# yynil/RWKV_LM_EXT

Measured on AMD Instinct MI355X. Metric: WKV6 fwd+bwd tokens/sec/GPU (B=8,T=4096,C=2048) + %HBM roofline, higher is better.
Workload: dtype bf16

## Files before the change

### rwkv_lm_ext_amd/csrc/wkv6_chunk.hip

```cpp
#include <type_traits>
#include "wkv6_chunk.h"

namespace wkv6 {
namespace {

using namespace chunk;

constexpr int GRP_BYTES = NBLK * BLK_BYTES;
constexpr int CKX_BYTES = 4 * 4096;
constexpr int CONSUMER_STAGGER = 3;
constexpr int YRS = 144;
constexpr int YS_BYTES = GRP * YRS;

struct FwdRaw {
    uint2 pr[4], pk[4], pv[4], pw[4];
    float4 pe[4];
};
template <bool W_RAW, bool STATE_ONLY, bool AFF>
__device__ __forceinline__ void fwd_request_group(const ScanArgs& a, const int b, const int h, const int ntok, const int rev, const int grp, const int wv,
                                                  const int lane, FwdRaw& raw)
{
    const int c4 = lane & 15, tq = lane >> 4;
    const long base = (long)b * a.T * a.C + (long)h * HEAD;
    const TokAddr<AFF> tok(ntok, rev != 0);
    const int C_ = a.C;
    const unsigned span = ntok > 0 ? (unsigned)(ntok - 1) * a.C : 0u;
    const unsigned nb2 = ntok > 0 ? span * 2 + 128 : 0;
    const rsrc_t rs_r = make_rsrc(reinterpret_cast<const bf16_t*>(a.r) + base, nb2), rs_k = make_rsrc(reinterpret_cast<const bf16_t*>(a.k) + base, nb2);
    const rsrc_t rs_v = make_rsrc(reinterpret_cast<const bf16_t*>(a.v) + base, nb2);
    const rsrc_t rs_w = W_RAW ? make_rsrc(reinterpret_cast<const bf16_t*>(a.w) + base, nb2)
                              : make_rsrc(reinterpret_cast<const float*>(a.w) + base, ntok > 0 ? span * 4 + 256 : 0);
#pragma unroll
    for (int tt = 0; tt < 4; ++tt) {
        const int pl = wv * BLK + 4 * tq + tt, lp = tok.lane(pl, 4 * c4, C_);
        if constexpr (!STATE_ONLY) raw.pr[tt] = buf_load8(rs_r, tok.off(grp * GRP, pl, 4 * c4, C_, REV_R, lp) * 2);
        else raw.pr[tt] = make_uint2(0u, 0u);
        raw.pk[tt] = buf_load8(rs_k, tok.off(grp * GRP, pl, 4 * c4, C_, REV_K, lp) * 2);
        raw.pv[tt] = buf_load8(rs_v, tok.off(grp * GRP, pl, 4 * c4, C_, REV_V, lp) * 2);
        if constexpr (W_RAW) raw.pw[tt] = buf_load8(rs_w, tok.off(grp * GRP, pl, 4 * c4, C_, REV_W, lp) * 2);
        else raw.pe[tt] = buf_load16f(rs_w, tok.off(grp * GRP, pl, 4 * c4, C_, REV_W, lp) * 4);
    }
}
struct FwdChain {
    int b, ntok;
    int pb;
    bool chained_in;
    bool nx_valid;
    unsigned nx_bh;
    int nx_b, nx_ntok;
    bool nx_rev, nx_use_u;
};
__device__ __forceinline__ bool fwd_hw_wave_produces(int hw) { return hw >= 4; }
template <bool W_RAW, bool STATE_ONLY, bool ACC, bool GN, bool AFF, bool CLK = false, bool CHAIN = false, bool VARLEN = false>
__device__ __forceinline__ void chunk_fwd_body(const ScanArgs& a, const unsigned slot, const unsigned sslot, FwdRaw& raw, const FwdChain& ch = FwdChain{})
{
    [[maybe_unused]] const bool nxvalid = ch.nx_valid, chained_in = ch.chained_in, nx_use_u = ch.nx_use_u;
    [[maybe_unused]] const unsigned nxbh = ch.nx_bh;
    [[maybe_unused]] const int nxrev = ch.nx_rev, b_known = ch.b, ntok_known = ch.ntok, nxb = ch.nx_b, nxntok = ch.nx_ntok, pb = CHAIN ? ch.pb : 0;
    extern __shared__ __attribute__((aligned(16))) char smem[];
    const int tid = threadIdx.x, lane = tid & 63;
    const SplitConst spc = split_const();
    const int hwid = __builtin_amdgcn_readfirstlane(tid >> 6);
    const int part = a.split ? (int)(slot & 1) : 0;
    const int bh = a.split ? (int)(slot >> 1) : (CLK ? (int)(slot + 0u * (unsigned)(a.B * a.H)) : (int)slot);
    int wid, cidx;
    wid = a.split ? (hwid < 2 ? 2 * part + hwid : hwid + 2) : hwid;
    cidx = hwid;
    const bool producer = wid >= 4;
    const int wv = wid & 3;
    const int b = CHAIN ? b_known : (a.order ? a.order[bh / a.H] : bh / a.H), h = bh % a.H;
    const long base = VARLEN ? (long)a.tok_off[b] * a.C + (long)h * HEAD : (long)b * a.T * a.C + (long)h * HEAD;
    const bf16_t* const gr_ = reinterpret_cast<const bf16_t*>(a.r) + base;
    const bf16_t* const gk_ = reinterpret_cast<const bf16_t*>(a.k) + base;
    const bf16_t* const gv_ = reinterpret_cast<const bf16_t*>(a.v) + base;
    bf16_t* const gy_ = reinterpret_cast<bf16_t*>(a.y) + base;
    int ntok = a.T;
    if constexpr (CHAIN) ntok = ntok_known;
    else if (a.lens) ntok = min(max(a.lens[b], 0), a.T);
    const int ngrp = (ntok + GRP - 1) / GRP;
    const TokAddr<AFF> tok(a, b, ntok);
    const int C_ = a.C;
#ifdef WKV6_STAMP
    unsigned long long stamp_acc[6] = {0, 0, 0, 0, 0, 0}, ts0 = 0, ts1 = 0, ts2 = 0, ts3 = 0, ts4 = 0;
#endif
#ifdef WKV6_DEBUGBUF
    unsigned long long clk0 = 0, rtc0 = 0, clk1 = 0, rtc1 = 0;
    WKV6_CLK(clk0, rtc0);
#endif
    if constexpr (CLK) { if (hwid == 0) clock_stamp(a, slot, 0); }

    if (producer) {
        const int c4 = lane & 15, tq = lane >> 4;
        float uu[4] = {0.f, 0.f, 0.f, 0.f};
        if (a.use_u) io4<bf16_t>::load(reinterpret_cast<const bf16_t*>(a.u) + h * HEAD + 4 * c4, uu);
        uint2 (&pr)[4] = raw.pr, (&pk)[4] = raw.pk, (&pv)[4] = raw.pv, (&pw)[4] = raw.pw;
        float4 (&pe)[4] = raw.pe;
        float dtot[4] = {0.f, 0.f, 0.f, 0.f};
        const unsigned span = ntok > 0 ? (unsigned)(ntok - 1) * a.C : 0u;
        const rsrc_t rs_r = make_rsrc(gr_, ntok > 0 ? span * 2 + 128 : 0), rs_k = make_rsrc(gk_, ntok > 0 ? span * 2 + 128 : 0);
        const rsrc_t rs_v = make_rsrc(gv_, ntok > 0 ? span * 2 + 128 : 0);
        const rsrc_t rs_w = W_RAW ? make_rsrc(reinterpret_cast<const bf16_t*>(a.w) + base, ntok > 0 ? span * 2 + 128 : 0)
                                  : make_rsrc(reinterpret_cast<const float*>(a.w) + base, ntok > 0 ? span * 4 + 256 : 0);
        const int lp_in[4] = {tok.lane(wv * BLK + 4 * tq, 4 * c4, C_), tok.lane(wv * BLK + 4 * tq + 1, 4 * c4, C_),
                              tok.lane(wv * BLK + 4 * tq + 2, 4 * c4, C_), tok.lane(wv * BLK + 4 * tq + 3, 4 * c4, C_)};
        auto load_quad = [&](int grp, int tt) {
            {
                const int pl = wv * BLK + 4 * tq + tt;
                const unsigned ir = tok.off(grp * GRP, pl, 4 * c4, C_, REV_R, lp_in[tt]), ik = tok.off(grp * GRP, pl, 4 * c4, C_, REV_K, lp_in[tt]);
                const unsigned iv = tok.off(grp * GRP, pl, 4 * c4, C_, REV_V, lp_in[tt]), iw = tok.off(grp * GRP, pl, 4 * c4, C_, REV_W, lp_in[tt]);
                if constexpr (!STATE_ONLY) pr[tt] = buf_load8(rs_r, ir * 2);
                else pr[tt] = make_uint2(0u, 0u);
                pk[tt] = buf_load8(rs_k, ik * 2);
                pv[tt] = buf_load8(rs_v, iv * 2);
                if constexpr (W_RAW) pw[tt] = buf_load8(rs_w, iw * 2);
                else pe[tt] = buf_load16f(rs_w, iw * 4);
            }
        };
        auto load_group = [&](int grp) {
#pragma unroll
            for (int tt = 0; tt < 4; ++tt) load_quad(grp, tt);
        };
        auto prep_group = [&](int grp, int buf, const int ntok, const float (&uu)[4], auto&& request_next) {
            char* const bb = smem + buf * GRP_BYTES + wv * BLK_BYTES;
            float r[4][4], k[4][4], cs[4][4];
#pragma unroll
            for (int tt = 0; tt < 4; ++tt) {
                const bool valid = grp * GRP + wv * BLK + 4 * tq + tt < ntok;
                r[tt][0] = bf_lo(pr[tt].x); r[tt][1] = bf_hi(pr[tt].x); r[tt][2] = bf_lo(pr[tt].y); r[tt][3] = bf_hi(pr[tt].y);
                k[tt][0] = bf_lo(pk[tt].x); k[tt][1] = bf_hi(pk[tt].x); k[tt][2] = bf_lo(pk[tt].y); k[tt][3] = bf_hi(pk[tt].y);
                float lw[4];
                if constexpr (W_RAW) {
                    lw[0] = -LOG2E * exp2_fast(LOG2E * bf_lo(pw[tt].x)); lw[1] = -LOG2E * exp2_fast(LOG2E * bf_hi(pw[tt].x));
                    lw[2] = -LOG2E * exp2_fast(LOG2E * bf_lo(pw[tt].y)); lw[3] = -LOG2E * exp2_fast(LOG2E * bf_hi(pw[tt].y));
                } else {
                    lw[0] = pe[tt].x; lw[1] = pe[tt].y; lw[2] = pe[tt].z; lw[3] = pe[tt].w;
                    if (a.wkind == 2) {
#pragma unroll
                        for (int c = 0; c < 4; ++c) lw[c] = __builtin_amdgcn_logf(lw[c]);
                    } else {
#pragma unroll
                        for (int c = 0; c < 4; ++c) lw[c] *= LOG2E;
                    }
                }
#pragma unroll
                for (int c = 0; c < 4; ++c) {
                    const float l = valid ? fmaxf(lw[c], LW_MIN2) : 0.f;
                    cs[tt][c] = tt ? cs[tt - 1][c] + l : l;
                }
                if constexpr (!STATE_ONLY) {
                    float part = 0.f;
#pragma unroll
                    for (int c = 0; c < 4; ++c) part = fmaf(r[tt][c] * uu[c], k[tt][c], part);
                    part = row_sum16(part);
                    if (c4 == 0) *reinterpret_cast<float*>(bb + OFF_COEF + (4 * tq + tt) * 4) = part;
                }
                *reinterpret_cast<uint2*>(bb + A_V * ARR + (4 * tq + tt) * RSB + 8 * c4) = pv[tt];
            }
            __builtin_amdgcn_sched_barrier(0);
            request_next();
            float pre[4], c8[4], c16[4];
#pragma unroll
            for (int c = 0; c < 4; ++c) {
                float a_, b_;
                rows16(cs[3][c], a_, b_);
                float pfx = (tq & 1) ? a_ : 0.f;
                halves32(a_ + b_, a_, b_);
                pfx += (tq & 2) ? a_ : 0.f;
                pre[c] = pfx;
                c8[c] = a_;
                c16[c] = a_ + b_;
                dtot[c] += c16[c];
            }
            if (tq == 0) {
                *reinterpret_cast<float4*>(bb + OFF_E8 + 16 * c4) =
                    make_float4(exp2_fast(c8[0]), exp2_fast(c8[1]), exp2_fast(c8[2]), exp2_fast(c8[3]));
                *reinterpret_cast<float4*>(bb + OFF_E16M8 + 16 * c4) =
                    make_float4(exp2_fast(c16[0] - c8[0]), exp2_fast(c16[1] - c8[1]), exp2_fast(c16[2] - c8[2]), exp2_fast(c16[3] - c8[3]));
            }
#pragma unroll
            for (int tt = 0; tt < 4; ++tt) {
                float rh[4], kh[4];
#pragma unroll
                for (int c = 0; c < 4; ++c) {
                    const float cex = tt ? pre[c] + cs[tt - 1][c] : pre[c];
                    const float cin = pre[c] + cs[tt][c];
                    rh[c] = r[tt][c] * exp2_fast(cex - c8[c]);
                    kh[c] = k[tt][c] * exp2_fast(c8[c] - cin);
                }
                char* const row = bb + (4 * tq + tt) * RSB + 8 * c4;
                uint2 hi, lo;
                if constexpr (!STATE_ONLY) {
                    split4(rh, hi, lo, spc);
                    *reinterpret_cast<uint2*>(row + A_RH * ARR) = hi; *reinterpret_cast<uint2*>(row + A_RL * ARR) = lo;
                }
                split4(kh, hi, lo, spc);
                *reinterpret_cast<uint2*>(row + A_KH * ARR) = hi; *reinterpret_cast<uint2*>(row + A_KL * ARR) = lo;
            }
            if constexpr (!STATE_ONLY) {
                const int x = lane & 15, g = lane >> 4;
                f4v sc = {0.f, 0.f, 0.f, 0.f};
#pragma unroll
                for (int s = 0; s < 2; ++s) {
                    const int off = x * RSB + (32 * s + 8 * g) * 2;
                    const b8v kh = ld_b8(bb + A_KH * ARR + off), kl = ld_b8(bb + A_KL * ARR + off);
                    const b8v rh = ld_b8(bb + A_RH * ARR + off), rl = ld_b8(bb + A_RL * ARR + off);
                    sc = mfma32(kh, rh, sc);
                    sc = mfma32(kh, rl, sc);
                    sc = mfma32(kl, rh, sc);
                }
                const float cf = *reinterpret_cast<const float*>(bb + OFF_COEF + x * 4);
                float scm[4];
#pragma unroll
                for (int q = 0; q < 4; ++q) {
                    const int bt = 4 * g + q;
                    scm[q] = bt < x ? sc[q] : (bt == x ? cf : 0.f);
                }
                uint2 sh, sl;
                split4(scm, sh, sl, spc);
                *reinterpret_cast<uint4*>(bb + OFF_SC + lane * 16) = make_uint4(sh.x, sh.y, sl.x, sl.y);
            }
        };

        float uu_nx[4] = {0.f, 0.f, 0.f, 0.f};
        if constexpr (CHAIN) { if (nxvalid && nx_use_u) io4<bf16_t>::load(reinterpret_cast<const bf16_t*>(a.u) + (nxbh % (unsigned)a.H) * HEAD + 4 * c4, uu_nx); }
        if (!(CHAIN && chained_in)) {
            if (ngrp > 0) {
                load_group(0);
                prep_group(0, pb & 1, ntok, uu, [&]() { load_group(1); });
            }
            __syncthreads();
        }
        for (int grp = 0; grp + 1 < ngrp; ++grp) {
            WKV6_T(ts0);
#ifdef WKV6_STAMP
            asm volatile("" :: "v"(pr[0].x), "v"(pk[0].x), "v"(pv[0].x), "v"(pw[0].x), "v"(pr[3].x), "v"(pk[3].x), "v"(pv[3].x),
                         "v"(pw[3].x));
#endif
            WKV6_T(ts1);
            prep_group(grp + 1, (grp + 1 + pb) & 1, ntok, uu, [&]() { load_group(grp + 2); });
            WKV6_T(ts2);
            WKV6_T(ts3);
            __syncthreads();
            WKV6_T(ts4);
            WKV6_ACC(0, ts1, ts0); WKV6_ACC(1, ts2, ts1); WKV6_ACC(2, ts3, ts2); WKV6_ACC(3, ts4, ts3);
        }
        if constexpr (CHAIN) {
            if (nxvalid) {
                const int nxh = (int)(nxbh % (unsigned)a.H);
                fwd_request_group<W_RAW, STATE_ONLY, AFF>(a, nxb, nxh, nxntok, nxrev, 0, wv, lane, raw);
                prep_group(0, (ngrp + pb) & 1, nxntok, uu_nx, [&]() { fwd_request_group<W_RAW, STATE_ONLY, AFF>(a, nxb, nxh, nxntok, nxrev, 1, wv, lane, raw); });
            }
        }
        if (ngrp > 0) __syncthreads();
        if (a.dsum && tq == 0 && part == 0)
            *reinterpret_cast<float4*>(a.dsum + ((long)(b * a.H + h) * 4 + wv) * HEAD + 4 * c4) = make_float4(dtot[0], dtot[1], dtot[2], dtot[3]);
    } else {
        const int x = lane & 15, g = lane >> 4;
        f4v St[4];
#pragma unroll
        for (int it = 0; it < 4; ++it) {
            float t4[4] = {0.f, 0.f, 0.f, 0.f};
            if (a.s0) {
                const long so_ = (long)b * a.s0_bstride + ((long)h * HEAD + 16 * wv + x) * HEAD + tile_ch(it) + 8 * g;
                if (a.state_f32) io4<float>::load(reinterpret_cast<const float*>(a.s0) + so_, t4);
                else io4<bf16_t>::load(reinterpret_cast<const bf16_t*>(a.s0) + so_, t4);
            }
            St[it] = f4v{t4[0], t4[1], t4[2], t4[3]};
            asm volatile("" : "+v"(St[it]));
        }
        int troff = (4 * g + (x >> 2)) * RSB + 8 * (x & 3);
        int trow = (4 * g + (x >> 2)) * RSB + 16 * (x & 3);
        const rsrc_t rs_y = make_rsrc(a.y ? gy_ : nullptr, (!STATE_ONLY && a.y && ntok > 0) ? (unsigned)(ntok - 1) * a.C * 2u + 128u : 0u);
        const unsigned nst = VARLEN ? (unsigned)ngrp : ((unsigned)a.T + CKPT_TOK - 1) / CKPT_TOK;
        const int segs = a.ckpt_segs > 1 ? a.ckpt_segs : 1;
        const long ck_slot0 = VARLEN ? (long)h * a.ck_stride + a.ck_off[b] : ((long)((b / segs) * a.H + h) * segs + b % segs) * nst;
        const rsrc_t rs_ck = make_rsrc(a.ckpt ? a.ckpt + ck_slot0 * (HEAD * HEAD) : nullptr, a.ckpt ? nst * 16384u : 0u);
        const unsigned ystr = a.side_compact ? (unsigned)HEAD : (unsigned)a.C;
        const unsigned ych = a.side_compact ? 16u * (unsigned)cidx : 16u * (unsigned)wv;
        const rsrc_t rs_yf = make_rsrc(a.y_f32 ? a.y_f32 + (a.side_compact ? (long)sslot * a.T * HEAD : base) : nullptr,
                                       (a.y_f32 && !STATE_ONLY && ntok > 0) ? (unsigned)(ntok - 1) * ystr * 4u + 256u : 0u);
        const int lp_y = tok.lane(x, 16 * wv + 4 * g, C_), lp_ys = tok.lane(x, (int)ych + 4 * g, (int)ystr);
        [[maybe_unused]] uint4 acc_cur[NBLK] = {}, acc_nxt[NBLK] = {};
        auto acc_request = [&](int grp_, uint4 (&dst)[NBLK]) {
#pragma unroll
            for (int blk = 0; blk < NBLK; ++blk) {
                const unsigned idx = tok.off(grp_ * GRP + blk * BLK, x, 16 * wv + 4 * g, C_, REV_Y, lp_y);
                if (a.y_f32) {
                    const float4 t = buf_load16f(rs_yf, tok.off(grp_ * GRP + blk * BLK, x, (int)ych + 4 * g, (int)ystr, REV_Y, lp_ys) * 4u);
                    dst[blk] = make_uint4(__float_as_uint(t.x), __float_as_uint(t.y), __float_as_uint(t.z), __float_as_uint(t.w));
                } else {
                    const uint2 t = buf_load8(rs_y, idx * 2u);
                    dst[blk] = make_uint4(t.x, t.y, 0u, 0u);
                }
            }
        };
        auto acc_add = [&](const uint4& r, float (&o)[4]) {
            if (a.y_f32) { o[0] += __uint_as_float(r.x); o[1] += __uint_as_float(r.y); o[2] += __uint_as_float(r.z); o[3] += __uint_as_float(r.w); }
            else { o[0] += bf_lo(r.x); o[1] += bf_hi(r.x); o[2] += bf_lo(r.y); o[3] += bf_hi(r.y); }
        };
        if constexpr (ACC) {
            acc_request(0, acc_cur);
#pragma unroll
            for (int blk = 0; blk < NBLK; ++blk) asm volatile("" : "+v"(acc_cur[blk].x), "+v"(acc_cur[blk].y), "+v"(acc_cur[blk].z), "+v"(acc_cur[blk].w));
        }
        float gn_y[NBLK][4], gn_ga[4] = {1.f, 1.f, 1.f, 1.f}, gn_be[4] = {0.f, 0.f, 0.f, 0.f};
        uint2 gn_g[NBLK];
        unsigned gn_off[NBLK];
        char* const gn_stat = smem + 2 * GRP_BYTES;
        char* const ckx = smem + 2 * GRP_BYTES + (GN ? 4096 : 0) + cidx * 4096;
        char* const ys = smem + 2 * GRP_BYTES + (GN ? 4096 : 0) + CKX_BYTES;
        const int ylsh = a.split ? 2 : 3;
        auto stage_y = [&](int grp_, int blk, uint2 yb) {
            *reinterpret_cast<uint2*>(ys + (grp_ & 1) * YS_BYTES + (BLK * blk + x) * YRS + 32 * cidx + 8 * g) = yb;
        };
        const int fl_chunk = lane & ((1 << ylsh) - 1);
        const int fl_row[2] = {(GRP >> (ylsh - 1)) * cidx + (lane >> ylsh), (GRP >> (ylsh - 1)) * cidx + (64 >> ylsh) + (lane >> ylsh)};
        const int lp_fl[2] = {tok.lane(fl_row[0], 32 * part + 8 * fl_chunk, C_), tok.lane(fl_row[1], 32 * part + 8 * fl_chunk, C_)};
        auto flush_y = [&](int grp_) {
#pragma unroll
            for (int i = 0; i < 2; ++i) {
                const int row = fl_row[i], chunk = fl_chunk;
                const uint4 v = *reinterpret_cast<const uint4*>(ys + (grp_ & 1) * YS_BYTES + row * YRS + 16 * chunk);
                const unsigned off = tok.off(grp_ * GRP, row, 32 * part + 8 * chunk, C_, REV_Y, lp_fl[i]) * 2u;
                buf_store16(rs_y, off, v);
            }
        };
        const unsigned gn_bytes = (GN && ntok > 0) ? (unsigned)(ntok - 1) * a.C * 2u + 128u : 0u;
        const rsrc_t rs_gate = make_rsrc(GN ? reinterpret_cast<const bf16_t*>(a.gn_gate) + base : nullptr, gn_bytes);
        const rsrc_t rs_out = make_rsrc(GN ? reinterpret_cast<bf16_t*>(a.gn_out) + base : nullptr, gn_bytes);
        if constexpr (GN) {
            io4<bf16_t>::load(reinterpret_cast<const bf16_t*>(a.gn_gamma) + h * HEAD + 16 * wv + 4 * g, gn_ga);
            io4<bf16_t>::load(reinterpret_cast<const bf16_t*>(a.gn_beta) + h * HEAD + 16 * wv + 4 * g, gn_be);
        }
        auto gn_finish = [&](int grp) {
            const char* const st = gn_stat + (grp & 1) * 2048;
#pragma unroll
            for (int blk = 0; blk < NBLK; ++blk) {
                float s1 = 0.f, s2 = 0.f;
#pragma unroll
                for (int ww = 0; ww < 4; ++ww) {
                    const float2 t = *reinterpret_cast<const float2*>(st + ((ww * NBLK + blk) * 16 + x) * 8);
                    s1 += t.x; s2 += t.y;
                }
                const float mean = s1 * (1.f / 64.f);
                const float var = fmaxf(fmaf(-mean, mean, s2 * (1.f / 64.f)), 0.f);
                const float rstd = rsqrtf(var + a.gn_eps);
                const float gt[4] = {bf_lo(gn_g[blk].x), bf_hi(gn_g[blk].x), bf_lo(gn_g[blk].y), bf_hi(gn_g[blk].y)};
                float o[4];
#pragma unroll
                for (int qq = 0; qq < 4; ++qq) o[qq] = fmaf((gn_y[blk][qq] - mean) * rstd, gn_ga[qq], gn_be[qq]) * gt[qq];
                buf_store8(rs_out, gn_off[blk], make_uint2(pack_bf2(o[0], o[1]), pack_bf2(o[2], o[3])));
                const int p = grp * GRP + blk * BLK + x;
                if (a.gn_stats && wv == 0 && g == 0 && p < ntok) {
                    float* const sp = a.gn_stats + (((long)b * a.T + tok.token(p, REV_Y)) * a.H + h) * 2;
                    sp[0] = mean; sp[1] = rstd;
                }
            }
        };
        if (!(CHAIN && chained_in)) __syncthreads();
        constexpr bool STAGE_Y = !STATE_ONLY && !GN;
        const bool staged = STAGE_Y && (ACC || !a.y_f32);
        for (int grp = 0; grp < ngrp; ++grp) {
            WKV6_T(ts0);
            for (int i_ = 0; i_ < cidx; ++i_) __builtin_amdgcn_s_sleep(CONSUMER_STAGGER);
            if (staged && grp > 0) flush_y(grp - 1);
            if constexpr (ACC) acc_request(grp + 1, acc_nxt);

            constexpr bool unrolled = GN || ACC;
            const int nb = unrolled ? NBLK : min(NBLK, (ntok - grp * GRP + BLK - 1) / BLK);
            constexpr int unroll_by = unrolled ? NBLK : 1;
#pragma unroll unroll_by
            for (int blk = 0; blk < nb; ++blk) {
                const char* const bb = smem + ((grp + pb) & 1) * GRP_BYTES + blk * BLK_BYTES;
                typedef unsigned v4u __attribute__((ext_vector_type(4)));
                v4u ckd[4];
                int ck_off = -1;
                if (a.ckpt && blk == 0) {
                    const unsigned st = (unsigned)grp;
#pragma unroll
                    for (int it = 0; it < 4; ++it)
#pragma unroll
                        for (int q = 0; q < 4; ++q)
                            *reinterpret_cast<float*>(ckx + ((x ^ (q << 2)) + 16 * (g & 1) + 256 * (g >> 1) + 64 * (q & 1) + 128 * (q >> 1)
                                                             + 32 * (it & 1) + 512 * (it >> 1)) * 4) = St[it][q];
#pragma unroll
                    for (int wb = 0; wb < 4; ++wb)
                        ckd[wb] = *reinterpret_cast<const v4u*>(ckx + (4 * ((g >> 1) ^ (x & 1)) + 8 * ((g & 1) ^ ((x >> 1) & 1)) + 16 * ((x >> 3) & 1)
                                                                       + 32 * ((x >> 2) & 1) + 64 * (x & 1) + 128 * ((x >> 1) & 1) + 256 * wb) * 4);
                    ck_off = (int)(st * 16384u + (((2 * (wv >> 1) + (g >> 1)) * 64 + 16 * (2 * (wv & 1) + (g & 1)) + x) * 16));
                }
                const s4v vf4 = tr_read(bb + A_V * ARR + troff + 32 * wv);
                const b8v vf = __builtin_bit_cast(b8v, __builtin_shufflevector(vf4, vf4, 0, 1, 2, 3, 4, 5, 6, 7));
                [[maybe_unused]] uint4 scp = {};
                [[maybe_unused]] float4 pm0[2] = {}, pm1[2] = {};
                [[maybe_unused]] b8v pzh[2] = {}, pzl[2] = {};
#pragma unroll
                for (int s = 0; s < 2; ++s) {
                    pm0[s] = *reinterpret_cast<const float4*>(bb + OFF_E8 + (32 * s + 8 * g) * 4);
                    pm1[s] = *reinterpret_cast<const float4*>(bb + OFF_E8 + (32 * s + 8 * g + 4) * 4);
                }
                if constexpr (!STATE_ONLY) {
                    scp = *reinterpret_cast<const uint4*>(bb + OFF_SC + lane * 16);
#pragma unroll
                    for (int s = 0; s < 2; ++s) {
                        const int off = x * RSB + (32 * s + 8 * g) * 2;
                        pzh[s] = ld_b8(bb + A_RH * ARR + off);
                        pzl[s] = ld_b8(bb + A_RL * ARR + off);
                    }
                }
                b8v pk8[4];
                float4 pdm[4];
#pragma unroll
                for (int it = 0; it < 4; ++it) {
                    pk8[it] = __builtin_bit_cast(b8v, __builtin_shufflevector(tr_read(bb + A_KH * ARR + trow + tile_tr(it)),
                                                                              tr_read(bb + A_KL * ARR + trow + tile_tr(it)), 0, 1, 2, 3, 4, 5, 6, 7));
                    pdm[it] = *reinterpret_cast<const float4*>(bb + OFF_E16M8 + (tile_ch(it) + 8 * g) * 4);
                }
                __builtin_amdgcn_sched_barrier(0);
                f4v Tt[4];
#pragma unroll
                for (int s = 0; s < 2; ++s) {
                    const float4 m0 = pm0[s], m1 = pm1[s];
                    Tt[2 * s] = f4v{St[2 * s][0] * m0.x, St[2 * s][1] * m0.y, St[2 * s][2] * m0.z, St[2 * s][3] * m0.w};
                    Tt[2 * s + 1] = f4v{St[2 * s + 1][0] * m1.x, St[2 * s + 1][1] * m1.y, St[2 * s + 1][2] * m1.z, St[2 * s + 1][3] * m1.w};
                }
                if constexpr (!STATE_ONLY) {
                    f4v yt = {0.f, 0.f, 0.f, 0.f};
                    yt = mfma32(vf, __builtin_bit_cast(b8v, scp), yt);
#pragma unroll
                    for (int s = 0; s < 2; ++s) {
                        const float t0[4] = {Tt[2 * s][0], Tt[2 * s][1], Tt[2 * s][2], Tt[2 * s][3]};
                        const float t1[4] = {Tt[2 * s + 1][0], Tt[2 * s + 1][1], Tt[2 * s + 1][2], Tt[2 * s + 1][3]};
                        uint2 h0, l0, h1, l1;
                        split4(t0, h0, l0, spc);
                        split4(t1, h1, l1, spc);
                        const b8v s_hi = __builtin_bit_cast(b8v, make_uint4(h0.x, h0.y, h1.x, h1.y));
                        const b8v s_lo = __builtin_bit_cast(b8v, make_uint4(l0.x, l0.y, l1.x, l1.y));
                        const b8v zh = pzh[s], zl = pzl[s];
                        yt = mfma32(s_hi, zh, yt);
                        yt = mfma32(s_hi, zl, yt);
                        yt = mfma32(s_lo, zh, yt);
                    }
                    {
                        const int p = grp * GRP + blk * BLK + x;
                        float o[4] = {yt[0], yt[1], yt[2], yt[3]};
                        if (!ACC && !a.y_f32) {
                            const unsigned off = tok.off(grp * GRP + blk * BLK, x, 16 * wv + 4 * g, C_, REV_Y, lp_y) * 2u;
                            const uint2 yb = make_uint2(pack_bf2(o[0], o[1]), pack_bf2(o[2], o[3]));
                            if constexpr (GN) buf_store8(rs_y, off, yb);
                            else stage_y(grp, blk, yb);
                            if constexpr (GN) {
                                const float yr[4] = {bf_lo(yb.x), bf_hi(yb.x), bf_lo(yb.y), bf_hi(yb.y)};
                                gn_off[blk] = off;
                                gn_g[blk] = buf_load8(rs_gate, off);
                                float s1 = 0.f, s2 = 0.f;
#pragma unroll
                                for (int qq = 0; qq < 4; ++qq) { gn_y[blk][qq] = yr[qq]; s1 += yr[qq]; s2 = fmaf(yr[qq], yr[qq], s2); }
                                const float two[4] = {s1, s2, 0.f, 0.f};
                                const float red = col_reduce(two);
                                if ((g & 1) == 0)
                                    *reinterpret_cast<float*>(gn_stat + (grp & 1) * 2048 + ((wv * NBLK + blk) * 16 + x) * 8 + (g >> 1) * 4) = red;
                            }
                        } else {
                            if constexpr (ACC) acc_add(acc_cur[blk], o);
                            if (!ACC && a.y_f32) buf_store16f(rs_yf, tok.off(grp * GRP + blk * BLK, x, (int)ych + 4 * g, (int)ystr, REV_Y, lp_ys) * 4u, o);
                            else stage_y(grp, blk, make_uint2(pack_bf2(o[0], o[1]), pack_bf2(o[2], o[3])));
                        }
                    }
                }
#pragma unroll
                for (int it = 0; it < 4; ++it) {
                    const f4v o = mfma32(pk8[it], vf, Tt[it]);
                    const float4 dm = pdm[it];
                    St[it][0] = dm.x * o[0];
                    St[it][1] = dm.y * o[1];
                    St[it][2] = dm.z * o[2];
                    St[it][3] = dm.w * o[3];
                }
                if (ck_off >= 0) {
#pragma unroll
                    for (int wb = 0; wb < 4; ++wb)
                        __builtin_amdgcn_raw_buffer_store_b128(ckd[wb], rs_ck, ck_off + wb * 4096, 0, 2 );
                }
            }
            if constexpr (ACC) {
#pragma unroll
                for (int blk = 0; blk < NBLK; ++blk) acc_cur[blk] = acc_nxt[blk];
            }
            WKV6_T(ts1);
            __syncthreads();
            WKV6_T(ts2);
            WKV6_ACC(0, ts1, ts0); WKV6_ACC(1, ts2, ts1);
            if constexpr (GN) gn_finish(grp);
        }
        if (staged && ngrp > 0) flush_y(ngrp - 1);
        if (a.s_out) {
            const long so_ = ((long)b * a.H + h) * HEAD * HEAD + (long)(16 * wv + x) * HEAD + 8 * g;
#pragma unroll
            for (int it = 0; it < 4; ++it) {
                const float t4[4] = {St[it][0], St[it][1], St[it][2], St[it][3]};
                if (a.state_f32) io4<float>::store(reinterpret_cast<float*>(a.s_out) + so_ + tile_ch(it), t4);
                else io4<bf16_t>::store(reinterpret_cast<bf16_t*>(a.s_out) + so_ + tile_ch(it), t4);
            }
        }
        if constexpr (CHAIN) {
#pragma unroll
            for (int tt = 0; tt < 4; ++tt) {
                asm volatile("" : "=v"(raw.pr[tt].x), "=v"(raw.pr[tt].y), "=v"(raw.pk[tt].x), "=v"(raw.pk[tt].y),
                                  "=v"(raw.pv[tt].x), "=v"(raw.pv[tt].y), "=v"(raw.pw[tt].x), "=v"(raw.pw[tt].y));
                asm volatile("" : "=v"(raw.pe[tt].x), "=v"(raw.pe[tt].y), "=v"(raw.pe[tt].z), "=v"(raw.pe[tt].w));
            }
        }
    }
#ifdef WKV6_DEBUGBUF
    WKV6_CLK(clk1, rtc1);
    if (a.aux && lane == 0) {
        unsigned long long* const d = reinterpret_cast<unsigned long long*>(a.aux) + ((long)bh * 16 + wid) * 8;
#ifdef WKV6_STAMP
        for (int i = 0; i < 6; ++i) d[i] = stamp_acc[i];
#else
        d[5] = (unsigned long long)__builtin_amdgcn_s_getreg((31 << 11) | 4) | ((unsigned long long)hwid << 32);
#endif
        d[6] = clk1 - clk0;
        d[7] = rtc1 - rtc0;
    }
#endif
    if constexpr (CLK) { if (hwid == 0) clock_stamp(a, slot, 1); }
    if (!STATE_ONLY && !ACC && a.zero_tail) {
        const float z[4] = {0.f, 0.f, 0.f, 0.f};
        for (int t = ntok + (tid >> 4); part == 0 && t < a.T; t += (int)(blockDim.x >> 4))
            io4<bf16_t>::store(gy_ + (unsigned)(t * a.C + 4 * (tid & 15)), z);
    }
}

template <bool W_RAW, bool STATE_ONLY, bool ACC, bool GN, bool AFF>
__global__ __launch_bounds__(512) void chunk_fwd_kernel(const ScanArgs a)
{
    FwdRaw raw;
    chunk_fwd_body<W_RAW, STATE_ONLY, ACC, GN, AFF, !STATE_ONLY && !ACC && !GN>(a, blockIdx.x, 0u, raw);
}

template <bool W_RAW, bool STATE_ONLY>
__global__ __launch_bounds__(512) void chunk_fwd_varlen_kernel(const ScanArgs a)
{
    FwdRaw raw;
    chunk_fwd_body<W_RAW, STATE_ONLY, false, false, true, false, false, true>(a, blockIdx.x, 0u, raw);
}

template <bool W_RAW>
__global__ __launch_bounds__(512) void chunk_fwd_pair_kernel(const ScanArgs a0, const ScanArgs a1)
{
    const unsigned n = (unsigned)(a0.B * a0.H);
    const bool second = blockIdx.x >= n;
    FwdRaw raw;
    chunk_fwd_body<W_RAW, false, false, false, false>(second ? a1 : a0, second ? blockIdx.x - n : blockIdx.x, 0u, raw);
}

template <bool W_RAW>
__global__ __launch_bounds__(512) void chunk_fwd_bi_kernel(const ScanArgs a1_, float* const ckpt2)
{
    const unsigned n = (unsigned)(a1_.B * a1_.H);
    const int H_ = a1_.H, T_ = a1_.T, use_u_ = a1_.use_u;
    const int* const order_ = a1_.order;
    const int* const lens_ = a1_.lens;
    FwdRaw raw;
    const bool producer_wave = fwd_hw_wave_produces((int)(threadIdx.x >> 6));
    const auto row_of = [&](unsigned it) { return it * gridDim.x + ((it & 1) ? gridDim.x - 1 - blockIdx.x : blockIdx.x); };
    const auto lookup = [&](unsigned row, int& b, int& ntok) {
        b = 0; ntok = 0;
        if (row < n) {
            b = order_ ? order_[row / H_] : (int)(row / H_);
            ntok = lens_ ? min(max(lens_[b], 0), T_) : T_;
        }
    };
    int b_cur, ntok_cur;
    lookup(row_of(0), b_cur, ntok_cur);
    int pb = 0;
    bool chained = false;
    for (unsigned it = 0; it * gridDim.x < n; ++it) {
        const unsigned row = row_of(it);
        if (row >= n) continue;
        const unsigned row_nx = row_of(it + 1);
        int b_nx, ntok_nx;
        lookup(row_nx, b_nx, ntok_nx);
        const int ngrp_cur = (ntok_cur + GRP - 1) / GRP;
        {
            ScanArgs a1;
            load_kernargs(a1);
            chunk_fwd_body<W_RAW, false, false, false, true, false, true>(a1, row, blockIdx.x, raw,
                                                                          FwdChain{b_cur, ntok_cur, pb, chained, true, row, b_cur, ntok_cur, true, false});
        }
        pb = (pb + ngrp_cur) & 1;
        if (!producer_wave) __builtin_amdgcn_fence(__ATOMIC_RELEASE, "workgroup");
        __syncthreads();
        if (!producer_wave) __builtin_amdgcn_fence(__ATOMIC_ACQUIRE, "workgroup");
        {
            ScanArgs a2;
            load_kernargs(a2);
            a2.reverse = 1; a2.use_u = 0; a2.accumulate = 1; a2.zero_tail = 0; a2.ckpt = ckpt2;
            chunk_fwd_body<W_RAW, false, true, false, true, false, true>(a2, row, blockIdx.x, raw,
                                                                         FwdChain{b_cur, ntok_cur, pb, true, row_nx < n, row_nx, b_nx, ntok_nx, false, use_u_ != 0});
        }
        pb = (pb + ngrp_cur) & 1;
        chained = true;
        __syncthreads();
        b_cur = b_nx; ntok_cur = ntok_nx;
    }
}

template <bool W_RAW, bool STATE_ONLY, bool ACC, bool GN, bool AFF> hipError_t launch_fwd_variant2(const ScanArgs& a, hipStream_t st)
{
    constexpr size_t lds = 2 * (size_t)GRP_BYTES + (GN ? 4096 : 0) + CKX_BYTES + 2 * YS_BYTES;
    static LdsAttrOnce attr;
    if (hipError_t e = attr.ensure(reinterpret_cast<const void*>(chunk_fwd_kernel<W_RAW, STATE_ONLY, ACC, GN, AFF>), lds)) return e;
    if (a.split) hipLaunchKernelGGL((chunk_fwd_kernel<W_RAW, STATE_ONLY, ACC, GN, AFF>), dim3(2 * a.B * a.H), dim3(384), lds, st, a);
    else hipLaunchKernelGGL((chunk_fwd_kernel<W_RAW, STATE_ONLY, ACC, GN, AFF>), dim3(a.B * a.H), dim3(512), lds, st, a);
    return hipGetLastError();
}
template <bool W_RAW, bool STATE_ONLY, bool ACC, bool GN = false> hipError_t launch_fwd_variant(const ScanArgs& a, hipStream_t st)
{
    if constexpr (!ACC && !GN) { if (a.rev_n) return launch_fwd_variant2<W_RAW, STATE_ONLY, false, false, false>(a, st); }
    else if (a.rev_n) return hipErrorNotSupported;
    return launch_fwd_variant2<W_RAW, STATE_ONLY, ACC, GN, true>(a, st);
}

}

static bool offsets_fit(const ScanArgs& a) { return a.wkind == 1 || ((long)a.T + 64) * a.C < (1L << 30); }

hipError_t launch_chunk_fwd(const ScanArgs& a_, hipStream_t st)
{
    if (!offsets_fit(a_)) return hipErrorInvalidValue;
    ScanArgs a = a_;
    a.split = want_split(a.B * a.H);
    a.clk = clock_claim(0, &a.clk_slots);
    attach_debug_buffer(a);
    const bool raw = a.wkind == 1;
    if (a.gn_out) {
        if (a.split || a.accumulate || a.y_f32 || a.zero_tail) return hipErrorNotSupported;
        return raw ? launch_fwd_variant<true, false, false, true>(a, st) : launch_fwd_variant<false, false, false, true>(a, st);
    }
    if (a.accumulate) return raw ? launch_fwd_variant<true, false, true>(a, st) : launch_fwd_variant<false, false, true>(a, st);
    return raw ? launch_fwd_variant<true, false, false>(a, st) : launch_fwd_variant<false, false, false>(a, st);
}

hipError_t launch_chunk_fwd_pair(const ScanArgs& a0_, const ScanArgs& a1_, hipStream_t st)
{
    if (!offsets_fit(a0_) || !offsets_fit(a1_)) return hipErrorInvalidValue;
    if (a0_.B != a1_.B || a0_.T != a1_.T || a0_.C != a1_.C || a0_.H != a1_.H || a0_.wkind != a1_.wkind) return hipErrorInvalidValue;
    const auto plain = [](const ScanArgs& a) { return !a.accumulate && !a.y_f32 && !a.zero_tail && !a.gn_out && !a.dsum && !a.ckpt_segs; };
    if (!plain(a0_) || !plain(a1_)) return hipErrorNotSupported;
    if (want_split(a0_.B * a0_.H)) {
        if (hipError_t e = launch_chunk_fwd(a0_, st)) return e;
        return launch_chunk_fwd(a1_, st);
    }
    ScanArgs a0 = a0_, a1 = a1_;
    a0.split = a1.split = 0;
    constexpr size_t lds = 2 * (size_t)GRP_BYTES + CKX_BYTES + 2 * YS_BYTES;
    static LdsAttrOnce attr_raw, attr_ew;
    if (a0.wkind == 1) {
        if (hipError_t e = attr_raw.ensure(reinterpret_cast<const void*>(chunk_fwd_pair_kernel<true>), lds)) return e;
        hipLaunchKernelGGL((chunk_fwd_pair_kernel<true>), dim3(2 * a0.B * a0.H), dim3(512), lds, st, a0, a1);
    } else {
        if (hipError_t e = attr_ew.ensure(reinterpret_cast<const void*>(chunk_fwd_pair_kernel<false>), lds)) return e;
        hipLaunchKernelGGL((chunk_fwd_pair_kernel<false>), dim3(2 * a0.B * a0.H), dim3(512), lds, st, a0, a1);
    }
    return hipGetLastError();
}

hipError_t launch_chunk_fwd_bi(const ScanArgs& a1_, const ScanArgs& a2_, int* slots, hipStream_t st)
{
    const int n = bi_slots(a1_.B * a1_.H);
    if (slots) *slots = n;
    if (!n || !a1_.y_f32 || a1_.gn_out || a1_.dsum || a1_.ckpt_segs) return hipErrorNotSupported;
    if (!offsets_fit(a1_)) return hipErrorInvalidValue;
    ScanArgs a1 = a1_, a2 = a2_;
    a1.split = a2.split = 0;
    a1.side_compact = a2.side_compact = 1;
    attach_debug_buffer(a1);
    attach_debug_buffer(a2);
    constexpr size_t lds = 2 * (size_t)GRP_BYTES + CKX_BYTES + 2 * YS_BYTES;
    static LdsAttrOnce attr_raw, attr_ew;
    if (a1.wkind == 1) {
        if (hipError_t e = attr_raw.ensure(reinterpret_cast<const void*>(chunk_fwd_bi_kernel<true>), lds)) return e;
        hipLaunchKernelGGL((chunk_fwd_bi_kernel<true>), dim3(n), dim3(512), lds, st, a1, a2.ckpt);
    } else {
        if (hipError_t e = attr_ew.ensure(reinterpret_cast<const void*>(chunk_fwd_bi_kernel<false>), lds)) return e;
        hipLaunchKernelGGL((chunk_fwd_bi_kernel<false>), dim3(n), dim3(512), lds, st, a1, a2.ckpt);
    }
    return hipGetLastError();
}

template <bool W_RAW, bool STATE_ONLY> static hipError_t launch_fwd_varlen_inst(const ScanArgs& a, hipStream_t st)
{
    constexpr size_t lds = 2 * (size_t)GRP_BYTES + CKX_BYTES + 2 * YS_BYTES;
    static LdsAttrOnce attr;
    if (hipError_t e = attr.ensure(reinterpret_cast<const void*>(chunk_fwd_varlen_kernel<W_RAW, STATE_ONLY>), lds)) return e;
    hipLaunchKernelGGL((chunk_fwd_varlen_kernel<W_RAW, STATE_ONLY>), dim3(a.B * a.H), dim3(512), lds, st, a);
    return hipGetLastError();
}
hipError_t launch_chunk_fwd_varlen(const ScanArgs& a_, bool state_only, hipStream_t st)
{
    if (!offsets_fit(a_)) return hipErrorInvalidValue;
    if (!a_.tok_off || !a_.ck_off || !a_.lens || !a_.order) return hipErrorInvalidValue;
    if (a_.reverse || a_.rev_n || a_.accumulate || a_.y_f32 || a_.zero_tail || a_.gn_out || a_.dsum || a_.ckpt_segs > 1 || a_.side_compact)
        return hipErrorNotSupported;
    ScanArgs a = a_;
    a.split = 0;
    a.clk = nullptr; a.clk_slots = 0;
    attach_debug_buffer(a);
    const bool raw = a.wkind == 1;
    if (state_only) return raw ? launch_fwd_varlen_inst<true, true>(a, st) : launch_fwd_varlen_inst<false, true>(a, st);
    return raw ? launch_fwd_varlen_inst<true, false>(a, st) : launch_fwd_varlen_inst<false, false>(a, st);
}

hipError_t launch_chunk_state_pass(const ScanArgs& a_, hipStream_t st)
{
    if (!offsets_fit(a_)) return hipErrorInvalidValue;
    ScanArgs a = a_;
    a.split = want_split(a.B * a.H);
    return a.wkind == 1 ? launch_fwd_variant<true, true, false>(a, st) : launch_fwd_variant<false, true, false>(a, st);
}

size_t chunk_ckpt_floats(int B, int T, int H)
{
    return (size_t)B * H * ((T + CKPT_TOK - 1) / CKPT_TOK) * HEAD * HEAD;
}

}
```

Measured before the change: 56.64 million.

## Split forward producer work across two wave halves per block with LDS tag handoff

Doubles the producer waves in the chunk forward kernel for non-accumulate, non-GN, non-chain variants. Each producer wave now prepares half of its 16-token block (two tokens per lane instead of four), and the decay prefix is rebased so each half is written independently. An LDS tag spin-wait then lets the scoring half run the score computation only after both halves are written. This targets the serial latency of producer prep, which gates the consumers, at the cost of more threads per block (768), extra register and scheduling pressure, a spin-wait handshake, and extra barriers for the dsum reduction.

```diff
diff --git a/rwkv_lm_ext_amd/csrc/wkv6_chunk.hip b/rwkv_lm_ext_amd/csrc/wkv6_chunk.hip
--- a/rwkv_lm_ext_amd/csrc/wkv6_chunk.hip
+++ b/rwkv_lm_ext_amd/csrc/wkv6_chunk.hip
@@ -11,14 +11,19 @@
 constexpr int CONSUMER_STAGGER = 3;
 constexpr int YRS = 144;
 constexpr int YS_BYTES = GRP * YRS;
+constexpr int HALF = BLK / 2;
+constexpr int HTOK = 2;
+constexpr int SCORE_HALF = 1;
+constexpr int OFF_TAG = OFF_E16;
 
 struct FwdRaw {
-    uint2 pr[4], pk[4], pv[4], pw[4];
-    float4 pe[4];
+    uint2 pr[2 * HTOK], pk[2 * HTOK], pv[2 * HTOK], pw[2 * HTOK];
+    float4 pe[2 * HTOK];
 };
-template <bool W_RAW, bool STATE_ONLY, bool AFF>
+template <int NPW> __device__ __forceinline__ constexpr int fwd_lane_token(int hf, int tq, int i) { return HALF * (NPW == 2 ? hf : i / HTOK) + HTOK * tq + i % HTOK; }
+template <bool W_RAW, bool STATE_ONLY, bool AFF, int NPW>
 __device__ __forceinline__ void fwd_request_group(const ScanArgs& a, const int b, const int h, const int ntok, const int rev, const int grp, const int wv,
-                                                  const int lane, FwdRaw& raw)
+                                                  const int hf, const int lane, FwdRaw& raw)
 {
     const int c4 = lane & 15, tq = lane >> 4;
     const long base = (long)b * a.T * a.C + (long)h * HEAD;
@@ -31,8 +36,8 @@
     const rsrc_t rs_w = W_RAW ? make_rsrc(reinterpret_cast<const bf16_t*>(a.w) + base, nb2)
                               : make_rsrc(reinterpret_cast<const float*>(a.w) + base, ntok > 0 ? span * 4 + 256 : 0);
 #pragma unroll
-    for (int tt = 0; tt < 4; ++tt) {
-        const int pl = wv * BLK + 4 * tq + tt, lp = tok.lane(pl, 4 * c4, C_);
+    for (int tt = 0; tt < HTOK * (3 - NPW); ++tt) {
+        const int pl = wv * BLK + fwd_lane_token<NPW>(hf, tq, tt), lp = tok.lane(pl, 4 * c4, C_);
         if constexpr (!STATE_ONLY) raw.pr[tt] = buf_load8(rs_r, tok.off(grp * GRP, pl, 4 * c4, C_, REV_R, lp) * 2);
         else raw.pr[tt] = make_uint2(0u, 0u);
         raw.pk[tt] = buf_load8(rs_k, tok.off(grp * GRP, pl, 4 * c4, C_, REV_K, lp) * 2);
@@ -50,10 +55,12 @@
     int nx_b, nx_ntok;
     bool nx_rev, nx_use_u;
 };
+__host__ __device__ constexpr int fwd_npw(bool acc, bool gn, bool chain) { return (acc || gn || chain) ? 1 : 2; }
 __device__ __forceinline__ bool fwd_hw_wave_produces(int hw) { return hw >= 4; }
 template <bool W_RAW, bool STATE_ONLY, bool ACC, bool GN, bool AFF, bool CLK = false, bool CHAIN = false, bool VARLEN = false>
 __device__ __forceinline__ void chunk_fwd_body(const ScanArgs& a, const unsigned slot, const unsigned sslot, FwdRaw& raw, const FwdChain& ch = FwdChain{})
 {
+    constexpr int NPW = fwd_npw(ACC, GN, CHAIN), NH = 3 - NPW, NI = NH * HTOK;
     [[maybe_unused]] const bool nxvalid = ch.nx_valid, chained_in = ch.chained_in, nx_use_u = ch.nx_use_u;
     [[maybe_unused]] const unsigned nxbh = ch.nx_bh;
     [[maybe_unused]] const int nxrev = ch.nx_rev, b_known = ch.b, ntok_known = ch.ntok, nxb = ch.nx_b, nxntok = ch.nx_ntok, pb = CHAIN ? ch.pb : 0;
@@ -68,6 +75,7 @@
     cidx = hwid;
     const bool producer = wid >= 4;
     const int wv = wid & 3;
+    const int hf = NPW == 2 ? wid >> 3 : 0;
     const int b = CHAIN ? b_known : (a.order ? a.order[bh / a.H] : bh / a.H), h = bh % a.H;
     const long base = VARLEN ? (long)a.tok_off[b] * a.C + (long)h * HEAD : (long)b * a.T * a.C + (long)h * HEAD;
     const bf16_t* const gr_ = reinterpret_cast<const bf16_t*>(a.r) + base;
@@ -88,24 +96,33 @@
     WKV6_CLK(clk0, rtc0);
 #endif
     if constexpr (CLK) { if (hwid == 0) clock_stamp(a, slot, 0); }
+    typedef volatile int __attribute__((address_space(3))) lds_vint;
+    if constexpr (!STATE_ONLY && NPW == 2) {
+        if (!(CHAIN && chained_in)) {
+            if (tid < 2 * NBLK) *(lds_vint*)(smem + (tid >> 2) * GRP_BYTES + (tid & 3) * BLK_BYTES + OFF_TAG) = 0;
+            __syncthreads();
+        }
+    }
 
     if (producer) {
         const int c4 = lane & 15, tq = lane >> 4;
         float uu[4] = {0.f, 0.f, 0.f, 0.f};
         if (a.use_u) io4<bf16_t>::load(reinterpret_cast<const bf16_t*>(a.u) + h * HEAD + 4 * c4, uu);
-        uint2 (&pr)[4] = raw.pr, (&pk)[4] = raw.pk, (&pv)[4] = raw.pv, (&pw)[4] = raw.pw;
-        float4 (&pe)[4] = raw.pe;
-        float dtot[4] = {0.f, 0.f, 0.f, 0.f};
+        uint2 (&pr)[2 * HTOK] = raw.pr, (&pk)[2 * HTOK] = raw.pk, (&pv)[2 * HTOK] = raw.pv, (&pw)[2 * HTOK] = raw.pw;
+        float4 (&pe)[2 * HTOK] = raw.pe;
+        float dtot[NH][4] = {};
+        auto ltok = [&](int i) { return fwd_lane_token<NPW>(hf, tq, i); };
         const unsigned span = ntok > 0 ? (unsigned)(ntok - 1) * a.C : 0u;
         const rsrc_t rs_r = make_rsrc(gr_, ntok > 0 ? span * 2 + 128 : 0), rs_k = make_rsrc(gk_, ntok > 0 ? span * 2 + 128 : 0);
         const rsrc_t rs_v = make_rsrc(gv_, ntok > 0 ? span * 2 + 128 : 0);
         const rsrc_t rs_w = W_RAW ? make_rsrc(reinterpret_cast<const bf16_t*>(a.w) + base, ntok > 0 ? span * 2 + 128 : 0)
                                   : make_rsrc(reinterpret_cast<const float*>(a.w) + base, ntok > 0 ? span * 4 + 256 : 0);
-        const int lp_in[4] = {tok.lane(wv * BLK + 4 * tq, 4 * c4, C_), tok.lane(wv * BLK + 4 * tq + 1, 4 * c4, C_),
-                              tok.lane(wv * BLK + 4 * tq + 2, 4 * c4, C_), tok.lane(wv * BLK + 4 * tq + 3, 4 * c4, C_)};
+        int lp_in[NI];
+#pragma unroll
+        for (int i = 0; i < NI; ++i) lp_in[i] = tok.lane(wv * BLK + ltok(i), 4 * c4, C_);
         auto load_quad = [&](int grp, int tt) {
             {
-                const int pl = wv * BLK + 4 * tq + tt;
+                const int pl = wv * BLK + ltok(tt);
                 const unsigned ir = tok.off(grp * GRP, pl, 4 * c4, C_, REV_R, lp_in[tt]), ik = tok.off(grp * GRP, pl, 4 * c4, C_, REV_K, lp_in[tt]);
                 const unsigned iv = tok.off(grp * GRP, pl, 4 * c4, C_, REV_V, lp_in[tt]), iw = tok.off(grp * GRP, pl, 4 * c4, C_, REV_W, lp_in[tt]);
                 if constexpr (!STATE_ONLY) pr[tt] = buf_load8(rs_r, ir * 2);
@@ -118,14 +135,14 @@
         };
         auto load_group = [&](int grp) {
 #pragma unroll
-            for (int tt = 0; tt < 4; ++tt) load_quad(grp, tt);
+            for (int tt = 0; tt < NI; ++tt) load_quad(grp, tt);
         };
         auto prep_group = [&](int grp, int buf, const int ntok, const float (&uu)[4], auto&& request_next) {
             char* const bb = smem + buf * GRP_BYTES + wv * BLK_BYTES;
-            float r[4][4], k[4][4], cs[4][4];
-#pragma unroll
-            for (int tt = 0; tt < 4; ++tt) {
-                const bool valid = grp * GRP + wv * BLK + 4 * tq + tt < ntok;
+            float r[NI][4], k[NI][4], cs[NI][4];
+#pragma unroll
+            for (int tt = 0; tt < NI; ++tt) {
+                const bool valid = grp * GRP + wv * BLK + ltok(tt) < ntok;
                 r[tt][0] = bf_lo(pr[tt].x); r[tt][1] = bf_hi(pr[tt].x); r[tt][2] = bf_lo(pr[tt].y); r[tt][3] = bf_hi(pr[tt].y);
                 k[tt][0] = bf_lo(pk[tt].x); k[tt][1] = bf_hi(pk[tt].x); k[tt][2] = bf_lo(pk[tt].y); k[tt][3] = bf_hi(pk[tt].y);
                 float lw[4];
@@ -145,49 +162,48 @@
 #pragma unroll
                 for (int c = 0; c < 4; ++c) {
                     const float l = valid ? fmaxf(lw[c], LW_MIN2) : 0.f;
-                    cs[tt][c] = tt ? cs[tt - 1][c] + l : l;
+                    cs[tt][c] = (tt % HTOK) ? cs[tt - 1][c] + l : l;
                 }
                 if constexpr (!STATE_ONLY) {
                     float part = 0.f;
 #pragma unroll
                     for (int c = 0; c < 4; ++c) part = fmaf(r[tt][c] * uu[c], k[tt][c], part);
                     part = row_sum16(part);
-                    if (c4 == 0) *reinterpret_cast<float*>(bb + OFF_COEF + (4 * tq + tt) * 4) = part;
-                }
-                *reinterpret_cast<uint2*>(bb + A_V * ARR + (4 * tq + tt) * RSB + 8 * c4) = pv[tt];
+                    if (c4 == 0) *reinterpret_cast<float*>(bb + OFF_COEF + ltok(tt) * 4) = part;
+                }
+                *reinterpret_cast<uint2*>(bb + A_V * ARR + ltok(tt) * RSB + 8 * c4) = pv[tt];
             }
             __builtin_amdgcn_sched_barrier(0);
             request_next();
-            float pre[4], c8[4], c16[4];
+#pragma unroll
+            for (int hh = 0; hh < NH; ++hh) {
+            const int hfx = NPW == 2 ? hf : hh;
+            float pre[4], tot[4];
 #pragma unroll
             for (int c = 0; c < 4; ++c) {
                 float a_, b_;
-                rows16(cs[3][c], a_, b_);
+                rows16(cs[HTOK * hh + HTOK - 1][c], a_, b_);
                 float pfx = (tq & 1) ? a_ : 0.f;
                 halves32(a_ + b_, a_, b_);
                 pfx += (tq & 2) ? a_ : 0.f;
-                pre[c] = pfx;
-                c8[c] = a_;
-                c16[c] = a_ + b_;
-                dtot[c] += c16[c];
-            }
-            if (tq == 0) {
-                *reinterpret_cast<float4*>(bb + OFF_E8 + 16 * c4) =
-                    make_float4(exp2_fast(c8[0]), exp2_fast(c8[1]), exp2_fast(c8[2]), exp2_fast(c8[3]));
-                *reinterpret_cast<float4*>(bb + OFF_E16M8 + 16 * c4) =
-                    make_float4(exp2_fast(c16[0] - c8[0]), exp2_fast(c16[1] - c8[1]), exp2_fast(c16[2] - c8[2]), exp2_fast(c16[3] - c8[3]));
-            }
-#pragma unroll
-            for (int tt = 0; tt < 4; ++tt) {
+                tot[c] = a_ + b_;
+                pre[c] = hfx ? pfx : pfx - tot[c];
+                dtot[hh][c] += tot[c];
+            }
+            if (tq == 0)
+                *reinterpret_cast<float4*>(bb + (hfx ? OFF_E16M8 : OFF_E8) + 16 * c4) =
+                    make_float4(exp2_fast(tot[0]), exp2_fast(tot[1]), exp2_fast(tot[2]), exp2_fast(tot[3]));
+#pragma unroll
+            for (int tt = HTOK * hh; tt < HTOK * hh + HTOK; ++tt) {
                 float rh[4], kh[4];
 #pragma unroll
                 for (int c = 0; c < 4; ++c) {
-                    const float cex = tt ? pre[c] + cs[tt - 1][c] : pre[c];
+                    const float cex = (tt % HTOK) ? pre[c] + cs[tt - 1][c] : pre[c];
                     const float cin = pre[c] + cs[tt][c];
-                    rh[c] = r[tt][c] * exp2_fast(cex - c8[c]);
-                    kh[c] = k[tt][c] * exp2_fast(c8[c] - cin);
-                }
-                char* const row = bb + (4 * tq + tt) * RSB + 8 * c4;
+                    rh[c] = r[tt][c] * exp2_fast(cex);
+                    kh[c] = k[tt][c] * exp2_fast(-cin);
+                }
+                char* const row = bb + ltok(tt) * RSB + 8 * c4;
                 uint2 hi, lo;
                 if constexpr (!STATE_ONLY) {
                     split4(rh, hi, lo, spc);
@@ -196,7 +212,23 @@
                 split4(kh, hi, lo, spc);
                 *reinterpret_cast<uint2*>(row + A_KH * ARR) = hi; *reinterpret_cast<uint2*>(row + A_KL * ARR) = lo;
             }
-            if constexpr (!STATE_ONLY) {
+            }
+            if constexpr (!STATE_ONLY && NPW == 2) {
+                lds_vint* const tagp = (lds_vint*)(bb + OFF_TAG);
+                asm volatile("" ::: "memory");
+                if (hf != SCORE_HALF) {
+                    if (lane == 0) *tagp = 1;
+                } else {
+                    unsigned spins = 0;
+                    while (__builtin_amdgcn_ballot_w64(*tagp != 1) != 0) {
+                        if (++spins > (1u << 22)) __builtin_trap();
+                        __builtin_amdgcn_s_sleep(1);
+                    }
+                    if (lane == 0) *tagp = 0;
+                }
+                asm volatile("" ::: "memory");
+            }
+            if (!STATE_ONLY && (NPW == 1 || hf == SCORE_HALF)) {
                 const int x = lane & 15, g = lane >> 4;
                 f4v sc = {0.f, 0.f, 0.f, 0.f};
 #pragma unroll
@@ -233,8 +265,8 @@
         for (int grp = 0; grp + 1 < ngrp; ++grp) {
             WKV6_T(ts0);
 #ifdef WKV6_STAMP
-            asm volatile("" :: "v"(pr[0].x), "v"(pk[0].x), "v"(pv[0].x), "v"(pw[0].x), "v"(pr[3].x), "v"(pk[3].x), "v"(pv[3].x),
-                         "v"(pw[3].x));
+            asm volatile("" :: "v"(pr[0].x), "v"(pk[0].x), "v"(pv[0].x), "v"(pw[0].x), "v"(pr[NI - 1].x), "v"(pk[NI - 1].x), "v"(pv[NI - 1].x),
+                         "v"(pw[NI - 1].x));
 #endif
             WKV6_T(ts1);
             prep_group(grp + 1, (grp + 1 + pb) & 1, ntok, uu, [&]() { load_group(grp + 2); });
@@ -247,13 +279,24 @@
         if constexpr (CHAIN) {
             if (nxvalid) {
                 const int nxh = (int)(nxbh % (unsigned)a.H);
-                fwd_request_group<W_RAW, STATE_ONLY, AFF>(a, nxb, nxh, nxntok, nxrev, 0, wv, lane, raw);
-                prep_group(0, (ngrp + pb) & 1, nxntok, uu_nx, [&]() { fwd_request_group<W_RAW, STATE_ONLY, AFF>(a, nxb, nxh, nxntok, nxrev, 1, wv, lane, raw); });
+                fwd_request_group<W_RAW, STATE_ONLY, AFF, NPW>(a, nxb, nxh, nxntok, nxrev, 0, wv, hf, lane, raw);
+                prep_group(0, (ngrp + pb) & 1, nxntok, uu_nx, [&]() { fwd_request_group<W_RAW, STATE_ONLY, AFF, NPW>(a, nxb, nxh, nxntok, nxrev, 1, wv, hf, lane, raw); });
             }
         }
         if (ngrp > 0) __syncthreads();
-        if (a.dsum && tq == 0 && part == 0)
-            *reinterpret_cast<float4*>(a.dsum + ((long)(b * a.H + h) * 4 + wv) * HEAD + 4 * c4) = make_float4(dtot[0], dtot[1], dtot[2], dtot[3]);
+        if constexpr (!CHAIN) {
+            if (a.dsum) {
+                float* const dx = reinterpret_cast<float*>(smem + wv * BLK_BYTES + OFF_E8);
+                if (NPW == 2 && hf == 0 && tq == 0) *reinterpret_cast<float4*>(dx + 4 * c4) = make_float4(dtot[0][0], dtot[0][1], dtot[0][2], dtot[0][3]);
+                __syncthreads();
+                if ((NPW == 1 || hf == 1) && tq == 0 && part == 0) {
+                    const float4 d0 = NPW == 2 ? *reinterpret_cast<const float4*>(dx + 4 * c4) : make_float4(dtot[0][0], dtot[0][1], dtot[0][2], dtot[0][3]);
+                    const float (&d1)[4] = dtot[NH - 1];
+                    *reinterpret_cast<float4*>(a.dsum + ((long)(b * a.H + h) * 4 + wv) * HEAD + 4 * c4) =
+                        make_float4(d0.x + d1[0], d0.y + d1[1], d0.z + d1[2], d0.w + d1[3]);
+                }
+            }
+        }
     } else {
         const int x = lane & 15, g = lane >> 4;
         f4v St[4];
@@ -503,9 +546,10 @@
                 else io4<bf16_t>::store(reinterpret_cast<bf16_t*>(a.s_out) + so_ + tile_ch(it), t4);
             }
         }
+        if constexpr (!CHAIN) { if (a.dsum) __syncthreads(); }
         if constexpr (CHAIN) {
 #pragma unroll
-            for (int tt = 0; tt < 4; ++tt) {
+            for (int tt = 0; tt < NI; ++tt) {
                 asm volatile("" : "=v"(raw.pr[tt].x), "=v"(raw.pr[tt].y), "=v"(raw.pk[tt].x), "=v"(raw.pk[tt].y),
                                   "=v"(raw.pv[tt].x), "=v"(raw.pv[tt].y), "=v"(raw.pw[tt].x), "=v"(raw.pw[tt].y));
                 asm volatile("" : "=v"(raw.pe[tt].x), "=v"(raw.pe[tt].y), "=v"(raw.pe[tt].z), "=v"(raw.pe[tt].w));
@@ -533,22 +577,23 @@
     }
 }
 
+constexpr int fwd_threads(int npw, bool split = false) { return 64 * ((split ? 2 : 4) + 4 * npw); }
 template <bool W_RAW, bool STATE_ONLY, bool ACC, bool GN, bool AFF>
-__global__ __launch_bounds__(512) void chunk_fwd_kernel(const ScanArgs a)
+__global__ __launch_bounds__(fwd_threads(fwd_npw(ACC, GN, false))) void chunk_fwd_kernel(const ScanArgs a)
 {
     FwdRaw raw;
     chunk_fwd_body<W_RAW, STATE_ONLY, ACC, GN, AFF, !STATE_ONLY && !ACC && !GN>(a, blockIdx.x, 0u, raw);
 }
 
 template <bool W_RAW, bool STATE_ONLY>
-__global__ __launch_bounds__(512) void chunk_fwd_varlen_kernel(const ScanArgs a)
+__global__ __launch_bounds__(fwd_threads(2)) void chunk_fwd_varlen_kernel(const ScanArgs a)
 {
     FwdRaw raw;
     chunk_fwd_body<W_RAW, STATE_ONLY, false, false, true, false, false, true>(a, blockIdx.x, 0u, raw);
 }
 
 template <bool W_RAW>
-__global__ __launch_bounds__(512) void chunk_fwd_pair_kernel(const ScanArgs a0, const ScanArgs a1)
+__global__ __launch_bounds__(fwd_threads(2)) void chunk_fwd_pair_kernel(const ScanArgs a0, const ScanArgs a1)
 {
     const unsigned n = (unsigned)(a0.B * a0.H);
     const bool second = blockIdx.x >= n;
@@ -557,7 +602,7 @@
 }
 
 template <bool W_RAW>
-__global__ __launch_bounds__(512) void chunk_fwd_bi_kernel(const ScanArgs a1_, float* const ckpt2)
+__global__ __launch_bounds__(fwd_threads(1)) void chunk_fwd_bi_kernel(const ScanArgs a1_, float* const ckpt2)
 {
     const unsigned n = (unsigned)(a1_.B * a1_.H);
     const int H_ = a1_.H, T_ = a1_.T, use_u_ = a1_.use_u;
@@ -613,8 +658,8 @@
     constexpr size_t lds = 2 * (size_t)GRP_BYTES + (GN ? 4096 : 0) + CKX_BYTES + 2 * YS_BYTES;
     static LdsAttrOnce attr;
     if (hipError_t e = attr.ensure(reinterpret_cast<const void*>(chunk_fwd_kernel<W_RAW, STATE_ONLY, ACC, GN, AFF>), lds)) return e;
-    if (a.split) hipLaunchKernelGGL((chunk_fwd_kernel<W_RAW, STATE_ONLY, ACC, GN, AFF>), dim3(2 * a.B * a.H), dim3(384), lds, st, a);
-    else hipLaunchKernelGGL((chunk_fwd_kernel<W_RAW, STATE_ONLY, ACC, GN, AFF>), dim3(a.B * a.H), dim3(512), lds, st, a);
+    if (a.split) hipLaunchKernelGGL((chunk_fwd_kernel<W_RAW, STATE_ONLY, ACC, GN, AFF>), dim3(2 * a.B * a.H), dim3(fwd_threads(fwd_npw(ACC, GN, false), true)), lds, st, a);
+    else hipLaunchKernelGGL((chunk_fwd_kernel<W_RAW, STATE_ONLY, ACC, GN, AFF>), dim3(a.B * a.H), dim3(fwd_threads(fwd_npw(ACC, GN, false))), lds, st, a);
     return hipGetLastError();
 }
 template <bool W_RAW, bool STATE_ONLY, bool ACC, bool GN = false> hipError_t launch_fwd_variant(const ScanArgs& a, hipStream_t st)
@@ -660,10 +705,10 @@
     static LdsAttrOnce attr_raw, attr_ew;
     if (a0.wkind == 1) {
         if (hipError_t e = attr_raw.ensure(reinterpret_cast<const void*>(chunk_fwd_pair_kernel<true>), lds)) return e;
-        hipLaunchKernelGGL((chunk_fwd_pair_kernel<true>), dim3(2 * a0.B * a0.H), dim3(512), lds, st, a0, a1);
+        hipLaunchKernelGGL((chunk_fwd_pair_kernel<true>), dim3(2 * a0.B * a0.H), dim3(fwd_threads(2)), lds, st, a0, a1);
     } else {
         if (hipError_t e = attr_ew.ensure(reinterpret_cast<const void*>(chunk_fwd_pair_kernel<false>), lds)) return e;
-        hipLaunchKernelGGL((chunk_fwd_pair_kernel<false>), dim3(2 * a0.B * a0.H), dim3(512), lds, st, a0, a1);
+        hipLaunchKernelGGL((chunk_fwd_pair_kernel<false>), dim3(2 * a0.B * a0.H), dim3(fwd_threads(2)), lds, st, a0, a1);
     }
     return hipGetLastError();
 }
@@ -683,10 +728,10 @@
     static LdsAttrOnce attr_raw, attr_ew;
     if (a1.wkind == 1) {
         if (hipError_t e = attr_raw.ensure(reinterpret_cast<const void*>(chunk_fwd_bi_kernel<true>), lds)) return e;
-        hipLaunchKernelGGL((chunk_fwd_bi_kernel<true>), dim3(n), dim3(512), lds, st, a1, a2.ckpt);
+        hipLaunchKernelGGL((chunk_fwd_bi_kernel<true>), dim3(n), dim3(fwd_threads(1)), lds, st, a1, a2.ckpt);
     } else {
         if (hipError_t e = attr_ew.ensure(reinterpret_cast<const void*>(chunk_fwd_bi_kernel<false>), lds)) return e;
-        hipLaunchKernelGGL((chunk_fwd_bi_kernel<false>), dim3(n), dim3(512), lds, st, a1, a2.ckpt);
+        hipLaunchKernelGGL((chunk_fwd_bi_kernel<false>), dim3(n), dim3(fwd_threads(1)), lds, st, a1, a2.ckpt);
     }
     return hipGetLastError();
 }
@@ -696,7 +741,7 @@
     constexpr size_t lds = 2 * (size_t)GRP_BYTES + CKX_BYTES + 2 * YS_BYTES;
     static LdsAttrOnce attr;
     if (hipError_t e = attr.ensure(reinterpret_cast<const void*>(chunk_fwd_varlen_kernel<W_RAW, STATE_ONLY>), lds)) return e;
-    hipLaunchKernelGGL((chunk_fwd_varlen_kernel<W_RAW, STATE_ONLY>), dim3(a.B * a.H), dim3(512), lds, st, a);
+    hipLaunchKernelGGL((chunk_fwd_varlen_kernel<W_RAW, STATE_ONLY>), dim3(a.B * a.H), dim3(fwd_threads(2)), lds, st, a);
     return hipGetLastError();
 }
 hipError_t launch_chunk_fwd_varlen(const ScanArgs& a_, bool state_only, hipStream_t st)
```

Result: no change. 56.37 million (-0.5%).
